# cmusphinx/pocketsphinx

Hardware: NVIDIA H100
Metric: frames/sec senone-eval+Viterbi (higher is better)
Workload: dtype f32->i16/i32

## Files before the change

### pocketsphinx_b200/csrc/psb_ptm_tc.cu

```cuda
#include "psb_gau.cuh"
#include "psb_internal.cuh"

#include <algorithm>
#include <cmath>
#include <cstring>

namespace {

constexpr int TC_ROWS = 128;
constexpr int TC_K = 32;
constexpr int TC_CAP = 18;
constexpr float TC_ERR = 1.0f / 262144.f;

enum {
    ST_ROWS, ST_FILTER_ALONE, ST_EXACT_DIST, ST_TIE_FLAGS,
    ST_OVER_CAP,
    ST_LANE_OVER,
    ST_FALLBACK_LISTED, ST_FALLBACK_ALL,
    ST_SPLIT,
    ST_FAIL_GAP, ST_FAIL_STRADDLE, ST_FAIL_SIGN, ST_FAIL_SAT,
    ST_N
};
constexpr size_t TC_CHECK_BYTES = 16 + 8 * ST_N;

__device__ __forceinline__ float to_tf32(float x)
{
    unsigned r;
    asm("cvt.rna.tf32.f32 %0, %1;" : "=r"(r) : "f"(x));
    return __uint_as_float(r);
}

struct Top5 {
    int s[5];
    unsigned c;
    int c4;
    int n;
};

__device__ __forceinline__ void top5_insert(Top5 &t, int s, int c)
{
    int p = 0;
#pragma unroll
    for (int j = 0; j < 5; ++j) p += (j < t.n && t.s[j] >= s) ? 1 : 0;
    if (p >= 5) return;
#pragma unroll
    for (int j = 4; j >= 1; --j)
        if (j > p) t.s[j] = t.s[j - 1];
#pragma unroll
    for (int j = 0; j < 5; ++j)
        if (j == p) t.s[j] = s;
    if (p < 4) {
        const unsigned lowmask = p == 0 ? 0u : (0xffffffffu >> (32 - 8 * p));
        t.c4 = (int)(t.c >> 24);
        t.c = (t.c & lowmask) | ((unsigned)c << (8 * p)) | ((t.c << 8) & ~(lowmask | (0xffu << (8 * p))));
    }
    else
        t.c4 = c;
    if (t.n < 5) ++t.n;
}

constexpr int WG_ROWS = 64;
constexpr int WG_SLOTS = (TC_CAP + 1) * WG_ROWS * 4;
constexpr int WG_EXTRA = WG_SLOTS * 8 + WG_ROWS * 4 * 4 + WG_ROWS * 4 + 2 * WG_ROWS * 4 + WG_ROWS * 20;

__device__ __forceinline__ uint64_t wgmma_desc(const void *p, unsigned lbo_bytes, unsigned sbo_bytes)
{
    const uint64_t a = (uint64_t)(((unsigned)__cvta_generic_to_shared(p) >> 4) & 0x3fffu);
    return a | ((uint64_t)((lbo_bytes >> 4) & 0x3fffu) << 16) | ((uint64_t)((sbo_bytes >> 4) & 0x3fffu) << 32);
}

template <int R>
__device__ __forceinline__ void wgmma_fence_regs(float (&d)[R])
{
#pragma unroll
    for (int i = 0; i < R; ++i) asm volatile("" : "+f"(d[i])::"memory");
}

__device__ __forceinline__ void warpgroup_bar(int id) { asm volatile("bar.sync %0, 128;" ::"r"(id) : "memory"); }

template <int N>
struct Wgmma;
#define PSB_ACC8(i) "+f"(d[i]), "+f"(d[i + 1]), "+f"(d[i + 2]), "+f"(d[i + 3]), "+f"(d[i + 4]), "+f"(d[i + 5]), "+f"(d[i + 6]), "+f"(d[i + 7])
template <> struct Wgmma<64> {
    static __device__ __forceinline__ void mma(float (&d)[32], uint64_t a, uint64_t b, int accumulate)
    {
        asm volatile("{\n.reg .pred p;\nsetp.ne.b32 p, %34, 0;\nwgmma.mma_async.sync.aligned.m64n64k8.f32.tf32.tf32 {"
        "%0,%1,%2,%3,%4,%5,%6,%7,%8,%9,%10,%11,%12,%13,%14,%15,%16,%17,%18,%19,%20,%21,%22,%23,%24,%25,%26,%27,%28,%29,"
        "%30,%31"
        "}, %32, %33, p, 1, 1;\n}\n"
        : PSB_ACC8(0), PSB_ACC8(8), PSB_ACC8(16), PSB_ACC8(24)
        : "l"(a), "l"(b), "r"(accumulate));
    }
};
template <> struct Wgmma<128> {
    static __device__ __forceinline__ void mma(float (&d)[64], uint64_t a, uint64_t b, int accumulate)
    {
        asm volatile("{\n.reg .pred p;\nsetp.ne.b32 p, %66, 0;\nwgmma.mma_async.sync.aligned.m64n128k8.f32.tf32.tf32 {"
        "%0,%1,%2,%3,%4,%5,%6,%7,%8,%9,%10,%11,%12,%13,%14,%15,%16,%17,%18,%19,%20,%21,%22,%23,%24,%25,%26,%27,%28,%29,"
        "%30,%31,%32,%33,%34,%35,%36,%37,%38,%39,%40,%41,%42,%43,%44,%45,%46,%47,%48,%49,%50,%51,%52,%53,%54,%55,%56,"
        "%57,%58,%59,%60,%61,%62,%63"
        "}, %64, %65, p, 1, 1;\n}\n"
        : PSB_ACC8(0), PSB_ACC8(8), PSB_ACC8(16), PSB_ACC8(24), PSB_ACC8(32), PSB_ACC8(40), PSB_ACC8(48), PSB_ACC8(56)
        : "l"(a), "l"(b), "r"(accumulate));
    }
};
template <> struct Wgmma<256> {
    static __device__ __forceinline__ void mma(float (&d)[128], uint64_t a, uint64_t b, int accumulate)
    {
        asm volatile("{\n.reg .pred p;\nsetp.ne.b32 p, %130, 0;\nwgmma.mma_async.sync.aligned.m64n256k8.f32.tf32.tf32 {"
        "%0,%1,%2,%3,%4,%5,%6,%7,%8,%9,%10,%11,%12,%13,%14,%15,%16,%17,%18,%19,%20,%21,%22,%23,%24,%25,%26,%27,%28,%29,"
        "%30,%31,%32,%33,%34,%35,%36,%37,%38,%39,%40,%41,%42,%43,%44,%45,%46,%47,%48,%49,%50,%51,%52,%53,%54,%55,%56,"
        "%57,%58,%59,%60,%61,%62,%63,%64,%65,%66,%67,%68,%69,%70,%71,%72,%73,%74,%75,%76,%77,%78,%79,%80,%81,%82,%83,"
        "%84,%85,%86,%87,%88,%89,%90,%91,%92,%93,%94,%95,%96,%97,%98,%99,%100,%101,%102,%103,%104,%105,%106,%107,%108,"
        "%109,%110,%111,%112,%113,%114,%115,%116,%117,%118,%119,%120,%121,%122,%123,%124,%125,%126,%127"
        "}, %128, %129, p, 1, 1;\n}\n"
        : PSB_ACC8(0), PSB_ACC8(8), PSB_ACC8(16), PSB_ACC8(24), PSB_ACC8(32), PSB_ACC8(40), PSB_ACC8(48), PSB_ACC8(56),
          PSB_ACC8(64), PSB_ACC8(72), PSB_ACC8(80), PSB_ACC8(88), PSB_ACC8(96), PSB_ACC8(104), PSB_ACC8(112),
          PSB_ACC8(120)
        : "l"(a), "l"(b), "r"(accumulate));
    }
};
#undef PSB_ACC8

template <int FL, int ND, bool CHECK>
__global__ void __launch_bounds__(2 * 128, 1)
ptm_wgmma_kernel(const float *__restrict__ feats, long long total, int D, const int32_t *__restrict__ featoff,
                 const int32_t *__restrict__ klist, const float *__restrict__ wumma, const float *__restrict__ cen,
                 const float *__restrict__ bnd, const float *__restrict__ rec, const size_t *__restrict__ rec_off,
                 int4 *__restrict__ out, unsigned *__restrict__ flags, long long flag_words, int K, int n_feat,
                 int tiles_per_cta, uint4 *__restrict__ items, unsigned *__restrict__ n_items, unsigned item_cap,
                 float *__restrict__ check, unsigned long long *__restrict__ stats)
{
    constexpr int RF = (1 + 2 * FL + 3) / 4 * 4;
    constexpr int NTL = ND / 8;
    constexpr int NPG = NTL / 8;
    constexpr unsigned FULL = 0xffffffffu;
    static_assert(2 * FL + 1 <= TC_K && (ND == 64 || ND == 128 || ND == 256), "shape");
    extern __shared__ __align__(128) unsigned char wg_smem[];
    const int tid = threadIdx.x, wg = tid >> 7, t = tid & 127, warp = t >> 5, lane = tid & 31;
    float *sW = reinterpret_cast<float *>(wg_smem);
    float *sX = sW + 2 * 8 * ND * 4 + wg * (2 * 8 * WG_ROWS * 4);
    unsigned char *ex = wg_smem + (size_t)2 * 8 * ND * 16 + 2 * (2 * 8 * WG_ROWS * 16) + (size_t)wg * WG_EXTRA;
    float2 *Pv = reinterpret_cast<float2 *>(ex);
    unsigned *Pm = reinterpret_cast<unsigned *>(Pv + WG_SLOTS);
    float *thrs = reinterpret_cast<float *>(Pm + WG_ROWS * 4);
    float *epsr = thrs + WG_ROWS;
    unsigned *Lc = reinterpret_cast<unsigned *>(epsr + 2 * WG_ROWS);

    const int k = klist[blockIdx.x];
    const int f = k % n_feat;
    {
        const float4 *src = reinterpret_cast<const float4 *>(wumma + (size_t)k * 2 * 8 * ND * 4);
        float4 *dst = reinterpret_cast<float4 *>(sW);
        for (int i = tid; i < 2 * 8 * ND; i += 2 * 128) dst[i] = src[i];
    }
    __syncthreads();
    const float *m = cen + (size_t)k * 16, *bb = bnd + (size_t)k * 32;
    const float *rc = rec + rec_off[k];
    const int r = t & (WG_ROWS - 1), half = t >> 6;
    const int g = lane >> 2, q4 = lane & 3;
    const int ra = warp * 16 + g, rb = ra + 8;

    float xn[FL];
    auto fetch = [&](long long row) {
        const float *p = feats + (row < total ? row : 0) * D + featoff[f];
#pragma unroll
        for (int j = 0; j < FL; ++j) xn[j] = row < total ? p[j] : 0.f;
    };
    auto prepare = [&](float *eps) {
        float v[TC_K];
        float S = bb[2 * FL];
#pragma unroll
        for (int j = 0; j < FL; ++j) {
            const float y = __fsub_rn(xn[j], m[j]);
            const float y2 = __fmul_rn(y, y);
            v[j] = y2;
            v[FL + j] = y;
            if (half == 0) {
                S = __fadd_ru(S, __fmul_ru(bb[j], y2));
                S = __fadd_ru(S, __fmul_ru(bb[FL + j], fabsf(y)));
            }
        }
        v[2 * FL] = 1.0f;
#pragma unroll
        for (int j = 2 * FL + 1; j < TC_K; ++j) v[j] = 0.f;
#pragma unroll
        for (int kc = 0; kc < 8; ++kc) {
            if ((kc & 1) != half) continue;
            float4 h, l;
            h.x = to_tf32(v[4 * kc]); h.y = to_tf32(v[4 * kc + 1]); h.z = to_tf32(v[4 * kc + 2]); h.w = to_tf32(v[4 * kc + 3]);
            l.x = to_tf32(__fsub_rn(v[4 * kc], h.x)); l.y = to_tf32(__fsub_rn(v[4 * kc + 1], h.y));
            l.z = to_tf32(__fsub_rn(v[4 * kc + 2], h.z)); l.w = to_tf32(__fsub_rn(v[4 * kc + 3], h.w));
            reinterpret_cast<float4 *>(sX)[kc * WG_ROWS + r] = h;
            reinterpret_cast<float4 *>(sX)[(8 + kc) * WG_ROWS + r] = l;
        }
        if (half == 0) eps[r] = __fadd_ru(__fmul_ru(S, TC_ERR), 2.0f);
        asm volatile("fence.proxy.async.shared::cta;" ::: "memory");
        warpgroup_bar(1 + wg);
    };
    float acc[ND / 2];
    auto gemm = [&]() {
#pragma unroll
        for (int i = 0; i < ND / 2; ++i) acc[i] = 0.f;
        wgmma_fence_regs(acc);
        asm volatile("wgmma.fence.sync.aligned;" ::: "memory");
#pragma unroll
        for (int pass = 0; pass < 3; ++pass) {
            const int ha = pass == 0 ? 1 : 0, hb = pass == 1 ? 1 : 0;
#pragma unroll
            for (int ks = 0; ks < 4; ++ks) {
                const uint64_t ad = wgmma_desc(sX + (size_t)(ha * 8 + 2 * ks) * WG_ROWS * 4, WG_ROWS * 16, 128);
                const uint64_t bd = wgmma_desc(sW + (size_t)(hb * 8 + 2 * ks) * ND * 4, ND * 16, 128);
                Wgmma<ND>::mma(acc, ad, bd, (pass | ks) ? 1 : 0);
            }
        }
        asm volatile("wgmma.commit_group.sync.aligned;" ::: "memory");
    };

    auto resolve = [&](const long long row0, const float *eps) {
        const int rr = t >> 1, h = t & 1;
        const long long row = row0 + rr;
        const bool valid = row < total;
        unsigned char *lb = reinterpret_cast<unsigned char *>(Lc + rr * 5);
        float a[5] = {-INFINITY, -INFINITY, -INFINITY, -INFINITY, -INFINITY};
        int c[5] = {0, 0, 0, 0, 0};
        int nl = 0;
        bool over = false;
        {
            const float thr = thrs[rr];
            auto cand = [&](float v, int col) {
                const bool p = v >= thr;
                if (p && nl < TC_CAP) lb[h ? TC_CAP - 1 - nl : nl] = (unsigned char)col;
                nl += p ? 1 : 0;
                v = p ? v : -INFINITY;
#pragma unroll
                for (int j = 0; j < 5; ++j) {
                    const bool s = v > a[j];
                    const float tv = a[j];
                    const int tc = c[j];
                    a[j] = s ? v : tv; c[j] = s ? col : tc;
                    v = s ? tv : v; col = s ? tc : col;
                }
            };
            unsigned m0 = Pm[rr * 4 + 2 * h], m1 = Pm[rr * 4 + 2 * h + 1];
            over = __popc(m0) > TC_CAP || __popc(m1) > TC_CAP;
            int j0 = 0, j1 = 0;
            while ((m0 | m1) != 0u) {
                const bool first = m0 != 0u;
                const unsigned msk = first ? m0 : m1;
                const int i = __ffs(msk) - 1, q = 2 * h + (first ? 0 : 1), j = first ? j0 : j1;
                const float2 v = Pv[j * WG_ROWS * 4 + rr * 4 + q];
                cand(v.x, 8 * i + 2 * q);
                cand(v.y, 8 * i + 2 * q + 1);
                if (first) { m0 = ++j0 < TC_CAP ? m0 & (m0 - 1u) : 0u; }
                else { m1 = ++j1 < TC_CAP ? m1 & (m1 - 1u) : 0u; }
            }
        }
        const int n1 = __shfl_xor_sync(FULL, nl, 1), n = nl + n1;
        over = __shfl_xor_sync(FULL, (int)over, 1) != 0 || over;
        {
            float b[5];
            int bc[5];
#pragma unroll
            for (int j = 0; j < 5; ++j) { b[j] = __shfl_xor_sync(FULL, a[j], 1); bc[j] = __shfl_xor_sync(FULL, c[j], 1); }
#pragma unroll
            for (int j = 0; j < 5; ++j)
                if (b[4 - j] > a[j]) { a[j] = b[4 - j]; c[j] = bc[4 - j]; }
            auto cmpx = [&](int i, int j) {
                if (a[j] > a[i]) { const float tv = a[i]; const int tc = c[i]; a[i] = a[j]; c[i] = c[j]; a[j] = tv; c[j] = tc; }
            };
            cmpx(0, 1); cmpx(3, 4); cmpx(2, 4); cmpx(2, 3); cmpx(1, 4); cmpx(0, 3); cmpx(0, 2); cmpx(1, 3); cmpx(1, 2);
        }
        const bool listed = n >= 5 && n <= TC_CAP && !over;
        const float ee = eps[rr];

        bool certain = listed;
        {
            const float gap = __fadd_ru(__fadd_ru(ee, ee), 1.0f);
            int qv[4];
            bool gap_ok = true, straddle_ok = true;
#pragma unroll
            for (int j = 0; j < 4; ++j) {
                gap_ok &= __fsub_rd(a[j], a[j + 1]) > gap;
                const int lo = __float2int_ru(__fsub_rd(a[j], ee)), hi = __float2int_ru(__fadd_ru(a[j], ee));
                straddle_ok &= (lo >> PSB_SENSCR_SHIFT) == (hi >> PSB_SENSCR_SHIFT);
                qv[j] = lo >> PSB_SENSCR_SHIFT;
            }
            const bool sign_ok = __fadd_ru(a[0], ee) < -2.0f, sat_ok = a[4] > -2.0e9f;
            certain &= gap_ok && straddle_ok && sign_ok && sat_ok;
            if (valid && h == 0) {
                if (CHECK) {
                    atomicMax(reinterpret_cast<int *>(check) + 1, n);
                    if (n > TC_CAP) atomicAdd(stats + ST_OVER_CAP, 1ull);
                    if (over) atomicAdd(stats + ST_LANE_OVER, 1ull);
                    if (listed) {
                        if (!gap_ok) atomicAdd(stats + ST_FAIL_GAP, 1ull);
                        if (!straddle_ok) atomicAdd(stats + ST_FAIL_STRADDLE, 1ull);
                        if (!sign_ok) atomicAdd(stats + ST_FAIL_SIGN, 1ull);
                        if (!sat_ok) atomicAdd(stats + ST_FAIL_SAT, 1ull);
                    }
                }
                if (certain) {
                    unsigned cb = 0, eb = 0;
#pragma unroll
                    for (int j = 0; j < 4; ++j) {
                        int ev = qv[0] - qv[j];
                        ev = ev > 255 ? 255 : ev;
                        cb |= (unsigned)c[j] << (8 * j);
                        eb |= (unsigned)ev << (8 * j);
                    }
                    out[row * K + k] = make_int4(qv[0], (int)cb, (int)eb, 0);
                    if (CHECK) { atomicAdd(stats, 1ull); atomicAdd(stats + 1, 1ull); }
                }
            }
        }
        __syncwarp();
        const bool doubt = valid && h == 0 && !certain;
        const int n0 = listed ? nl : 255, nb = listed ? n1 : 0;
        if (CHECK && doubt && listed && nl > 0 && n1 > 0) atomicAdd(stats + ST_SPLIT, 1ull);
        bool handled = false;
        if (items) {
            const unsigned need = __ballot_sync(FULL, doubt);
            if (need) {
                const int leader = __ffs(need) - 1;
                unsigned base = 0;
                if (lane == leader) base = atomicAdd(n_items, (unsigned)__popc(need));
                base = __shfl_sync(FULL, base, leader);
                const unsigned slot = base + (unsigned)__popc(need & ((1u << lane) - 1u));
                if (doubt && slot < item_cap) {
                    const unsigned *w = Lc + rr * 5;
                    items[2 * (size_t)slot] = make_uint4((unsigned)row, (unsigned)k | ((unsigned)n0 << 16) | ((unsigned)nb << 24), w[0], w[1]);
                    items[2 * (size_t)slot + 1] = make_uint4(w[2], w[3], w[4], (unsigned)(row >> 32));
                    handled = true;
                    if (CHECK) atomicAdd(stats, 1ull);
                }
            }
        }
        if (doubt && !handled) {
            float x[FL];
            const float *px = feats + row * D + featoff[f];
#pragma unroll
            for (int j = 0; j < FL; ++j) x[j] = px[j];
            Top5 top;
            top.n = 0; top.c = 0u; top.c4 = 0;
#pragma unroll
            for (int j = 0; j < 5; ++j) top.s[j] = INT_MIN;
            const int cnt_l = listed ? n : ND;
            if (CHECK) atomicAdd(stats + (listed ? ST_FALLBACK_LISTED : ST_FALLBACK_ALL), 1ull);
            for (int i = 0; i < cnt_l; ++i) {
                const int cw = listed ? (int)lb[i < n0 ? i : i - n0 + TC_CAP - nb] : i;
                const float d = gau_dist<FL>(reinterpret_cast<const float4 *>(rc + (size_t)cw * RF), x);
                top5_insert(top, f2i_clamped(d), cw);
            }
            const bool distinct = top.n >= 5 && top.s[0] > top.s[1] && top.s[1] > top.s[2] && top.s[2] > top.s[3] && top.s[3] > top.s[4];
            const int tp = top.s[0] >> PSB_SENSCR_SHIFT;
            unsigned eb = 0;
#pragma unroll
            for (int j = 0; j < 4; ++j) {
                int ev = tp - (top.s[j] >> PSB_SENSCR_SHIFT);
                ev = ev > 255 ? 255 : ev;
                eb |= (unsigned)ev << (8 * j);
            }
            out[row * K + k] = make_int4(tp, (int)top.c, (int)eb, 0);
            if (!distinct) atomicOr(&flags[(size_t)k * flag_words + (row >> 5)], 1u << (row & 31));
            if (CHECK) { atomicAdd(stats, 1ull); atomicAdd(stats + 2, (unsigned long long)cnt_l); if (!distinct) atomicAdd(stats + 3, 1ull); }
        }
    };

    long long row0 = (long long)blockIdx.y * tiles_per_cta * TC_ROWS + wg * WG_ROWS;
    if (row0 >= total) return;
    fetch(row0 + r);
    prepare(epsr);
    int buf = 0;
    for (int tile = 0;; ++tile, buf ^= 1, row0 += TC_ROWS) {
        gemm();
        const bool more = tile + 1 < tiles_per_cta && row0 + TC_ROWS < total;
        if (more) fetch(row0 + TC_ROWS + r);
        if (tile > 0) {
            resolve(row0 - TC_ROWS, epsr + (buf ^ 1) * WG_ROWS);
            warpgroup_bar(1 + wg);
        }
        const float *eps = epsr + buf * WG_ROWS;
        asm volatile("wgmma.wait_group.sync.aligned 0;" ::: "memory");
        wgmma_fence_regs(acc);

        float gma[8], gmb[8];
#pragma unroll
        for (int q = 0; q < 8; ++q) {
            float a = -INFINITY, b = -INFINITY;
#pragma unroll
            for (int i = q * NPG; i < (q + 1) * NPG; ++i) {
                a = fmaxf(fmaxf(a, acc[4 * i]), acc[4 * i + 1]);
                b = fmaxf(fmaxf(b, acc[4 * i + 2]), acc[4 * i + 3]);
            }
            a = fmaxf(a, __shfl_xor_sync(FULL, a, 1)); a = fmaxf(a, __shfl_xor_sync(FULL, a, 2));
            b = fmaxf(b, __shfl_xor_sync(FULL, b, 1)); b = fmaxf(b, __shfl_xor_sync(FULL, b, 2));
            gma[q] = a; gmb[q] = b;
        }
        auto fifth = [](float (&gm)[8]) {
            auto cmpx = [&](int i, int j) { const float hi = fmaxf(gm[i], gm[j]); gm[j] = fminf(gm[i], gm[j]); gm[i] = hi; };
#pragma unroll
            for (int o = 0; o < 8; o += 4) { cmpx(o, o + 1); cmpx(o + 2, o + 3); cmpx(o, o + 2); cmpx(o + 1, o + 3); cmpx(o + 1, o + 2); }
            return fmaxf(fmaxf(fminf(gm[0], gm[7]), fminf(gm[1], gm[6])), fmaxf(fminf(gm[2], gm[5]), fminf(gm[3], gm[4])));
        };
        const float e_a = eps[ra], e_b = eps[rb];
        const float thra = __fsub_rd(__fsub_rd(floorf(__fsub_rd(fifth(gma), e_a)), 1.0f), e_a);
        const float thrb = __fsub_rd(__fsub_rd(floorf(__fsub_rd(fifth(gmb), e_b)), 1.0f), e_b);
        {
            constexpr int SS = WG_ROWS * 4;
            int oa = ra * 4 + q4, ob = rb * 4 + q4;
            const int lim_a = oa + TC_CAP * SS, lim_b = ob + TC_CAP * SS;
            unsigned ma = 0u, mb = 0u;
#pragma unroll
            for (int i = 0; i < NTL; ++i) {
                const bool pa = fmaxf(acc[4 * i], acc[4 * i + 1]) >= thra;
                const bool pb = fmaxf(acc[4 * i + 2], acc[4 * i + 3]) >= thrb;
                if (pa) Pv[oa] = make_float2(acc[4 * i], acc[4 * i + 1]);
                if (pb) Pv[ob] = make_float2(acc[4 * i + 2], acc[4 * i + 3]);
                oa = pa ? min(oa + SS, lim_a) : oa;
                ob = pb ? min(ob + SS, lim_b) : ob;
                ma |= pa ? 1u << i : 0u;
                mb |= pb ? 1u << i : 0u;
            }
            Pm[ra * 4 + q4] = ma;
            Pm[rb * 4 + q4] = mb;
            if (q4 == 0) { thrs[ra] = thra; thrs[rb] = thrb; }
        }
        if (CHECK) {
            float worst = 0.f;
#pragma unroll
            for (int h = 0; h < 2; ++h) {
                const int rr = h ? rb : ra;
                if (row0 + rr >= total) continue;
                const float *px = feats + (row0 + rr) * D + featoff[f];
                const float er = eps[rr];
#pragma unroll
                for (int i = 0; i < NTL; ++i)
#pragma unroll
                    for (int e = 0; e < 2; ++e) {
                        const float *rp = rc + (size_t)(8 * i + 2 * q4 + e) * RF;
                        float d = rp[0];
                        for (int j = 0; j < FL; ++j) {
                            const float df = __fsub_rn(px[j], rp[1 + 2 * j]);
                            d = __fsub_rn(d, __fmul_rn(__fmul_rn(df, df), rp[2 + 2 * j]));
                        }
                        worst = fmaxf(worst, __fdividef(fabsf(acc[4 * i + 2 * h + e] - d), er));
                    }
            }
            atomicMax(reinterpret_cast<int *>(check), __float_as_int(worst));
        }
        warpgroup_bar(1 + wg);
        if (!more) break;
        prepare(epsr + (buf ^ 1) * WG_ROWS);
    }
    resolve(row0, epsr + buf * WG_ROWS);
}

template <int FL>
__global__ void __launch_bounds__(128)
ptm_tc_exact_kernel(const float *__restrict__ feats, int D, const int32_t *__restrict__ featoff, const uint4 *__restrict__ items,
                    const unsigned *__restrict__ n_items, unsigned item_cap, const float *__restrict__ rec,
                    const size_t *__restrict__ rec_off, int4 *__restrict__ out, unsigned *__restrict__ flags, long long flag_words,
                    int K, int n_feat, int nd, unsigned long long *__restrict__ stats)
{
    constexpr int RF = (1 + 2 * FL + 3) / 4 * 4;
    const unsigned count = min(*n_items, item_cap);
    for (unsigned i = blockIdx.x * blockDim.x + threadIdx.x; i < count; i += gridDim.x * blockDim.x) {
        const uint4 a = items[2 * (size_t)i], b = items[2 * (size_t)i + 1];
        const long long row = (long long)a.x | ((long long)b.w << 32);
        const int k = (int)(a.y & 0xffffu), n0 = (int)((a.y >> 16) & 0xffu), n1 = (int)(a.y >> 24);
        const unsigned wv[5] = {a.z, a.w, b.x, b.y, b.z};
        const float *px = feats + row * D + featoff[k % n_feat];
        const float *rc = rec + rec_off[k];
        float x[FL];
#pragma unroll
        for (int j = 0; j < FL; ++j) x[j] = px[j];
        Top5 top;
        top.n = 0; top.c = 0u; top.c4 = 0;
#pragma unroll
        for (int j = 0; j < 5; ++j) top.s[j] = INT_MIN;
        const int cnt = n0 == 255 ? nd : n0 + n1;
        for (int q = 0; q < cnt; ++q) {
            const int pos = q < n0 ? q : q - n0 + TC_CAP - n1;
            const int cw = n0 == 255 ? q : (int)((wv[pos >> 2] >> (8 * (pos & 3))) & 0xffu);
            const float d = gau_dist<FL>(reinterpret_cast<const float4 *>(rc + (size_t)cw * RF), x);
            top5_insert(top, f2i_clamped(d), cw);
        }
        const bool distinct = top.n >= 5 && top.s[0] > top.s[1] && top.s[1] > top.s[2] && top.s[2] > top.s[3] && top.s[3] > top.s[4];
        const int tp = top.s[0] >> PSB_SENSCR_SHIFT;
        unsigned eb = 0;
#pragma unroll
        for (int j = 0; j < 4; ++j) {
            int ev = tp - (top.s[j] >> PSB_SENSCR_SHIFT);
            ev = ev > 255 ? 255 : ev;
            eb |= (unsigned)ev << (8 * j);
        }
        out[row * K + k] = make_int4(tp, (int)top.c, (int)eb, 0);
        if (!distinct) atomicOr(&flags[(size_t)k * flag_words + (row >> 5)], 1u << (row & 31));
        if (stats) { atomicAdd(stats + 2, (unsigned long long)cnt); if (!distinct) atomicAdd(stats + 3, 1ull); }
    }
}

template <int FL, int NDW>
__global__ void __launch_bounds__(128)
ptm_fixup_warp_kernel(const float *__restrict__ feats, int D, const int32_t *__restrict__ featoff, const int32_t *__restrict__ utt_off,
                      int n_utt, const float *__restrict__ rec, const size_t *__restrict__ rec_off, int4 *__restrict__ out,
                      const unsigned *__restrict__ flags, long long flag_words, int K, int n_feat)
{
    constexpr int RF = (1 + 2 * FL + 3) / 4 * 4;
    constexpr unsigned FULL = 0xffffffffu;
    const long long id = ((long long)blockIdx.x * blockDim.x + threadIdx.x) >> 5;
    const int lane = threadIdx.x & 31;
    if (id >= (long long)n_utt * K) return;
    const int u = (int)(id / K), k = (int)(id % K);
    const int f = k % n_feat;
    const long long f0 = utt_off[u], f1 = utt_off[u + 1];
    if (f1 <= f0) return;
    const unsigned *fl = flags + (size_t)k * flag_words;
    const float *rc = rec + rec_off[k];
    for (long long w0 = f0 >> 5; w0 <= (f1 - 1) >> 5; w0 += 32) {
        const long long wd_l = w0 + lane;
        unsigned mine = wd_l <= ((f1 - 1) >> 5) ? fl[wd_l] : 0u;
        unsigned any = __ballot_sync(FULL, mine != 0u);
        while (any) {
            const int wl = __ffs(any) - 1;
            any &= any - 1;
            unsigned bits = __shfl_sync(FULL, mine, wl);
            while (bits) {
                const int b = __ffs(bits) - 1;
                bits &= bits - 1;
                const long long row = (w0 + wl) * 32 + b;
                if (row < f0 || row >= f1) continue;
                const float *px = feats + row * D + featoff[f];
                float x[FL];
#pragma unroll
                for (int j = 0; j < FL; ++j) x[j] = px[j];
                float d[NDW];
#pragma unroll
                for (int q = 0; q < NDW; ++q) d[q] = gau_dist<FL>(reinterpret_cast<const float4 *>(rc + (size_t)(lane + 32 * q) * RF), x);
                auto dist_of = [&](int c) {
                    float v = d[0];
#pragma unroll
                    for (int q = 1; q < NDW; ++q) v = (c >> 5) == q ? d[q] : v;
                    return __shfl_sync(FULL, v, c & 31);
                };
                const unsigned seeds = row == f0 ? 0x03020100u : (unsigned)out[(row - 1) * K + k].y;
                int cw[4], sc[4];
#pragma unroll
                for (int i = 0; i < 4; ++i) {
                    const int c = (seeds >> (8 * i)) & 0xff;
                    const int s = f2i_clamped(dist_of(c));
                    int p = 0;
#pragma unroll
                    for (int j = 0; j < i; ++j) p += (s > sc[j]) ? 0 : 1;
#pragma unroll
                    for (int j = 2; j >= 0; --j)
                        if (j < i && j >= p) { sc[j + 1] = sc[j]; cw[j + 1] = cw[j]; }
#pragma unroll
                    for (int j = 0; j < 4; ++j)
                        if (j == p) { sc[j] = s; cw[j] = c; }
                }
                const float th0 = (float)sc[3];
#pragma unroll
                for (int q = 0; q < NDW; ++q) {
                    unsigned cand = __ballot_sync(FULL, d[q] >= th0);
                    while (cand) {
                        const int l = __ffs(cand) - 1;
                        cand &= cand - 1;
                        const int c = l + 32 * q;
                        const float dv = __shfl_sync(FULL, d[q], l);
                        if (!(dv >= (float)sc[3])) continue;
                        if (cw[0] == c || cw[1] == c || cw[2] == c || cw[3] == c) continue;
                        const int s = f2i_clamped(dv);
                        int p = 0;
#pragma unroll
                        for (int j = 0; j < 3; ++j) p += (s >= sc[j]) ? 0 : 1;
#pragma unroll
                        for (int j = 2; j >= 0; --j)
                            if (j >= p) { sc[j + 1] = sc[j]; cw[j + 1] = cw[j]; }
#pragma unroll
                        for (int j = 0; j < 4; ++j)
                            if (j == p) { sc[j] = s; cw[j] = c; }
                    }
                }
                if (lane == 0) {
                    const int tp = sc[0] >> PSB_SENSCR_SHIFT;
                    unsigned cb = 0, eb = 0;
#pragma unroll
                    for (int j = 0; j < 4; ++j) {
                        int ev = tp - (sc[j] >> PSB_SENSCR_SHIFT);
                        ev = ev > 255 ? 255 : ev;
                        cb |= (unsigned)cw[j] << (8 * j);
                        eb |= (unsigned)ev << (8 * j);
                    }
                    out[row * K + k] = make_int4(tp, (int)cb, (int)eb, 0);
                }
                __syncwarp();
            }
        }
    }
}

float round_tf32_host(float x)
{
    uint32_t u;
    memcpy(&u, &x, 4);
    if ((u & 0x7f800000u) == 0x7f800000u) return x;
    u = (u + 0x1000u) & ~0x1fffu;
    float r;
    memcpy(&r, &u, 4);
    return r;
}

template <int FL, int ND>
int launch_wgmma(psb_batch_t *b, const float *d_feats, long long total, const int32_t *d_klist, int n_k, const int32_t *d_featoff,
               bool check)
{
    psb_model_t *m = b->m;
    const size_t smem = (size_t)2 * 8 * ND * 16 + 2 * ((size_t)2 * 8 * WG_ROWS * 16 + WG_EXTRA);
    const long long tiles = (total + TC_ROWS - 1) / TC_ROWS;
    const int n_sm = psb_sm_count(m->device);
    int per_sm = 1;
    PSB_CUDA(cudaFuncSetAttribute(ptm_wgmma_kernel<FL, ND, false>, cudaFuncAttributeMaxDynamicSharedMemorySize, (int)smem));
    PSB_CUDA(cudaOccupancyMaxActiveBlocksPerMultiprocessor(&per_sm, ptm_wgmma_kernel<FL, ND, false>, TC_ROWS * 2, smem));
    int tpc = 1;
    while (tpc < 32 && (tiles / (tpc * 2)) * n_k >= (long long)n_sm * std::max(per_sm, 1) * 4) tpc *= 2;
    PSB_REQUIRE((tiles + tpc - 1) / tpc <= 65535, "too many frames for one launch of the tensor-core filter");
    const dim3 grid((unsigned)n_k, (unsigned)((tiles + tpc - 1) / tpc));
    b->tc_last_tpc = tpc;
    b->tc_last_ctas = grid.y;
    float *chk = b->d_tc_check;
    unsigned long long *stats = reinterpret_cast<unsigned long long *>(b->d_tc_check + 4);
    if (check) {
        auto kern = ptm_wgmma_kernel<FL, ND, true>;
        PSB_CUDA(cudaFuncSetAttribute(kern, cudaFuncAttributeMaxDynamicSharedMemorySize, (int)smem));
        kern<<<grid, TC_ROWS * 2, smem, b->stream>>>(d_feats, total, m->sumlen, d_featoff, d_klist, m->d_tc_wumma, m->d_tc_cen, m->d_tc_bnd,
                                                m->d_rec, m->d_rec_off, b->d_topn, b->d_tc_flags, (long long)b->tc_flag_words, m->K,
                                                m->n_feat, tpc, b->d_tc_items, b->d_tc_nitems, b->tc_item_cap, chk, stats);
    }
    else {
        auto kern = ptm_wgmma_kernel<FL, ND, false>;
        PSB_CUDA(cudaFuncSetAttribute(kern, cudaFuncAttributeMaxDynamicSharedMemorySize, (int)smem));
        kern<<<grid, TC_ROWS * 2, smem, b->stream>>>(d_feats, total, m->sumlen, d_featoff, d_klist, m->d_tc_wumma, m->d_tc_cen, m->d_tc_bnd,
                                                m->d_rec, m->d_rec_off, b->d_topn, b->d_tc_flags, (long long)b->tc_flag_words, m->K,
                                                m->n_feat, tpc, b->d_tc_items, b->d_tc_nitems, b->tc_item_cap, nullptr, nullptr);
    }
    PSB_LAUNCH_CHECK();
    if (b->d_tc_items) {
        const unsigned blocks = (unsigned)std::min<size_t>(((size_t)b->tc_item_cap + 127) / 128, (size_t)n_sm * 64);
        ptm_tc_exact_kernel<FL><<<blocks, 128, 0, b->stream>>>(d_feats, m->sumlen, d_featoff, b->d_tc_items, b->d_tc_nitems, b->tc_item_cap,
                                                              m->d_rec, m->d_rec_off, b->d_topn, b->d_tc_flags, (long long)b->tc_flag_words,
                                                              m->K, m->n_feat, ND, check ? stats : nullptr);
        PSB_LAUNCH_CHECK();
    }
    return PSB_OK;
}

}

int psb_tc_prepare(psb_model_t *m, const float *hm, const float *hv, const float *hd)
{
    m->tc_ok = false;
    if (m->kind != PSB_KIND_PTM || m->fixed_point || m->topn != 4) return PSB_OK;
    if (m->n_density != 64 && m->n_density != 128 && m->n_density != 256) return PSB_OK;
    for (int f = 0; f < m->n_feat; ++f)
        if (m->featlen[f] != 13) return PSB_OK;
    const int nd = m->n_density, FL = 13, K = m->K;
    std::vector<float> cen((size_t)K * 16, 0.f), bnd((size_t)K * 32, 0.f);
    std::vector<float> wu((size_t)K * 2 * 8 * nd * 4, 0.f);
    std::vector<double> W((size_t)TC_K * nd);
    for (int cb = 0; cb < m->n_mgau; ++cb)
        for (int f = 0; f < m->n_feat; ++f) {
            const int k = cb * m->n_feat + f;
            const size_t src = ((size_t)cb * m->sumlen + m->featoff[f]) * nd;
            const float *mu = hm + src, *vv = hv + src, *dt = hd + (size_t)k * nd;
            float *c = cen.data() + (size_t)k * 16, *bb = bnd.data() + (size_t)k * 32;
            for (int j = 0; j < FL; ++j) {
                double s = 0;
                for (int q = 0; q < nd; ++q) s += mu[(size_t)q * FL + j];
                c[j] = (float)(s / nd);
            }
            std::fill(W.begin(), W.end(), 0.0);
            double cmax = 0;
            for (int q = 0; q < nd; ++q) {
                double c0 = dt[q], quad = 0;
                for (int j = 0; j < FL; ++j) {
                    const double v = vv[(size_t)q * FL + j], mp = (double)mu[(size_t)q * FL + j] - (double)c[j];
                    W[(size_t)j * nd + q] = -v;
                    W[(size_t)(FL + j) * nd + q] = 2.0 * v * mp;
                    quad += std::fabs(v) * mp * mp;
                    c0 -= v * mp * mp;
                    bb[j] = std::max(bb[j], (float)std::fabs(v));
                    bb[FL + j] = std::max(bb[FL + j], (float)std::fabs(2.0 * v * mp));
                }
                W[(size_t)(2 * FL) * nd + q] = c0;
                cmax = std::max(cmax, std::fabs((double)dt[q]) + quad);
            }
            bb[2 * FL] = (float)(cmax * 1.0001);
            for (int j = 0; j < 2 * FL; ++j) bb[j] = std::nextafter(bb[j] * 1.0001f, INFINITY);
            float *u = wu.data() + (size_t)k * 2 * 8 * nd * 4;
            for (int kk = 0; kk < TC_K; ++kk)
                for (int q = 0; q < nd; ++q) {
                    const float v = (float)W[(size_t)kk * nd + q], h = round_tf32_host(v);
                    u[((size_t)(kk >> 2) * nd + q) * 4 + (kk & 3)] = h;
                    u[((size_t)(8 + (kk >> 2)) * nd + q) * 4 + (kk & 3)] = round_tf32_host(v - h);
                }
            for (int i = 0; i < 32; ++i)
                if (!std::isfinite(bb[i])) return PSB_OK;
        }
    if (!m->d_tc_wumma) {
        PSB_CUDA(cudaMalloc(&m->d_tc_wumma, wu.size() * sizeof(float)));
        PSB_CUDA(cudaMalloc(&m->d_tc_cen, cen.size() * sizeof(float)));
        PSB_CUDA(cudaMalloc(&m->d_tc_bnd, bnd.size() * sizeof(float)));
    }
    PSB_CUDA(cudaMemcpy(m->d_tc_wumma, wu.data(), wu.size() * sizeof(float), cudaMemcpyHostToDevice));
    PSB_CUDA(cudaMemcpy(m->d_tc_cen, cen.data(), cen.size() * sizeof(float), cudaMemcpyHostToDevice));
    PSB_CUDA(cudaMemcpy(m->d_tc_bnd, bnd.data(), bnd.size() * sizeof(float), cudaMemcpyHostToDevice));
    m->tc_ok = true;
    return PSB_OK;
}

bool psb_tc_usable(const psb_batch_t *b)
{
    const psb_model_t *m = b->m;
    return m->tc_ok && m->ds_ratio == 1 && b->topn_variant >= 6;
}

int psb_launch_ptm_tc(psb_batch_t *b, const float *d_feats, const int32_t *utt_off, int32_t n_utt, const int32_t *d_klist,
                      const int32_t *d_featoff)
{
    psb_model_t *m = b->m;
    const long long total = utt_off[n_utt];
    const size_t fw = (size_t)((total + 31) / 32) + 1;
    if (fw * m->K > b->tc_flag_cap) {
        cudaFree(b->d_tc_flags);
        b->d_tc_flags = nullptr;
        b->tc_flag_cap = fw * m->K + fw * m->K / 8;
        PSB_CUDA(cudaMalloc(&b->d_tc_flags, b->tc_flag_cap * 4));
    }
    if ((size_t)n_utt + 1 > b->uttoff_cap) {
        if (b->d_uttoff) cudaFree(b->d_uttoff);
        b->d_uttoff = nullptr;
        b->uttoff_cap = (size_t)n_utt + 1 + 64;
        PSB_CUDA(cudaMalloc(&b->d_uttoff, b->uttoff_cap * sizeof(int32_t)));
    }
    if (!b->d_tc_check) {
        PSB_CUDA(cudaMalloc(&b->d_tc_check, TC_CHECK_BYTES));
        PSB_CUDA(cudaMemsetAsync(b->d_tc_check, 0, TC_CHECK_BYTES, b->stream));
    }
    {
        const size_t want = std::max<size_t>(4096, (size_t)total * m->K / 4);
        if (want > b->tc_item_cap || !b->d_tc_items) {
            cudaFree(b->d_tc_items);
            b->d_tc_items = nullptr;
            if (!b->d_tc_nitems) PSB_CUDA(cudaMalloc(&b->d_tc_nitems, 4));
            b->tc_item_cap = (unsigned)std::min<size_t>(want + want / 8, 0x7fffffffu);
            PSB_CUDA(cudaMalloc(&b->d_tc_items, (size_t)b->tc_item_cap * 32));
        }
        PSB_CUDA(cudaMemsetAsync(b->d_tc_nitems, 0, 4, b->stream));
    }
    b->tc_flag_words = fw;
    PSB_CUDA(cudaMemsetAsync(b->d_tc_flags, 0, fw * m->K * 4, b->stream));
    PSB_CUDA(cudaMemcpyAsync(b->d_uttoff, utt_off, ((size_t)n_utt + 1) * sizeof(int32_t), cudaMemcpyHostToDevice, b->stream));
    static const bool check = [] { const char *v = getenv("PSB_TC_CHECK"); return v && atoi(v) != 0; }();
    int rc;
    switch (m->n_density) {
    case 256: rc = launch_wgmma<13, 256>(b, d_feats, total, d_klist, m->K, d_featoff, check); break;
    case 128: rc = launch_wgmma<13, 128>(b, d_feats, total, d_klist, m->K, d_featoff, check); break;
    default: rc = launch_wgmma<13, 64>(b, d_feats, total, d_klist, m->K, d_featoff, check); break;
    }
    if (rc) return rc;
    const long long chains = (long long)n_utt * m->K;
    const unsigned blocks = (unsigned)((chains * 32 + 127) / 128);
#define PSB_FIXW(NDW) ptm_fixup_warp_kernel<13, NDW><<<blocks, 128, 0, b->stream>>>(d_feats, m->sumlen, d_featoff, b->d_uttoff, n_utt, \
        m->d_rec, m->d_rec_off, b->d_topn, b->d_tc_flags, (long long)fw, m->K, m->n_feat)
    if (m->n_density == 256) PSB_FIXW(8);
    else if (m->n_density == 128) PSB_FIXW(4);
    else PSB_FIXW(2);
#undef PSB_FIXW
    PSB_LAUNCH_CHECK();
    return PSB_OK;
}

extern "C" int psb_batch_tc_check(psb_batch_t *b, float *ratio, int32_t *max_candidates, int64_t *stats4)
{
    PSB_REQUIRE(b && ratio && max_candidates, "psb_batch_tc_check: null argument");
    *ratio = 0.f; *max_candidates = 0;
    if (stats4) stats4[0] = stats4[1] = stats4[2] = stats4[3] = 0;
    if (!b->d_tc_check) return PSB_OK;
    PSB_CUDA(cudaSetDevice(b->m->device));
    PSB_CUDA(cudaStreamSynchronize(b->stream));
    unsigned char h[64];
    PSB_CUDA(cudaMemcpy(h, b->d_tc_check, sizeof(h), cudaMemcpyDeviceToHost));
    memcpy(ratio, h, 4);
    memcpy(max_candidates, h + 4, 4);
    if (stats4) memcpy(stats4, h + 16, 32);
    return PSB_OK;
}

extern "C" int psb_batch_tc_counters(psb_batch_t *b, int64_t *out, int32_t n)
{
    PSB_REQUIRE(b && (out || n == 0) && n >= 0, "psb_batch_tc_counters: bad argument");
    static_assert(ST_N + 2 == PSB_TC_N_COUNTERS, "psb200.h lists every counter");
    int64_t v[PSB_TC_N_COUNTERS] = {0};
    if (b->d_tc_check) {
        PSB_CUDA(cudaSetDevice(b->m->device));
        PSB_CUDA(cudaStreamSynchronize(b->stream));
        PSB_CUDA(cudaMemcpy(v, reinterpret_cast<unsigned char *>(b->d_tc_check) + 16, 8 * ST_N, cudaMemcpyDeviceToHost));
    }
    v[ST_N] = b->tc_last_tpc;
    v[ST_N + 1] = b->tc_last_ctas;
    memcpy(out, v, sizeof(int64_t) * (size_t)std::min<int32_t>(n, PSB_TC_N_COUNTERS));
    return PSB_OK;
}
```

Baseline: 9.948 million.

## Use three warpgroups per CTA for small-ND tensor-core filter kernel

The wgmma filter kernel now launches a variable number of warpgroups per CTA: three when ND ≤ 128, two otherwise. Each warpgroup strides over 64-row half-tiles by the warpgroup count instead of owning a fixed half of every 128-row tile. Shared memory, the weight copy loop and the launch config are sized to match. The aim is more concurrent MMA and resolve work per SM, since the per-CTA weight tile is shared, at the cost of more shared memory and registers per CTA and possibly uneven work across warpgroups.

```diff
diff --git a/pocketsphinx_b200/csrc/psb_ptm_tc.cu b/pocketsphinx_b200/csrc/psb_ptm_tc.cu
--- a/pocketsphinx_b200/csrc/psb_ptm_tc.cu
+++ b/pocketsphinx_b200/csrc/psb_ptm_tc.cu
@@ -59,6 +59,7 @@
     if (t.n < 5) ++t.n;
 }
 
+__host__ __device__ constexpr int tc_warpgroups(int nd) { return nd > 128 ? 2 : 3; }
 constexpr int WG_ROWS = 64;
 constexpr int WG_SLOTS = (TC_CAP + 1) * WG_ROWS * 4;
 constexpr int WG_EXTRA = WG_SLOTS * 8 + WG_ROWS * 4 * 4 + WG_ROWS * 4 + 2 * WG_ROWS * 4 + WG_ROWS * 20;
@@ -123,7 +124,7 @@
 #undef PSB_ACC8
 
 template <int FL, int ND, bool CHECK>
-__global__ void __launch_bounds__(2 * 128, 1)
+__global__ void __launch_bounds__(tc_warpgroups(ND) * 128, 1)
 ptm_wgmma_kernel(const float *__restrict__ feats, long long total, int D, const int32_t *__restrict__ featoff,
                  const int32_t *__restrict__ klist, const float *__restrict__ wumma, const float *__restrict__ cen,
                  const float *__restrict__ bnd, const float *__restrict__ rec, const size_t *__restrict__ rec_off,
@@ -134,13 +135,14 @@
     constexpr int RF = (1 + 2 * FL + 3) / 4 * 4;
     constexpr int NTL = ND / 8;
     constexpr int NPG = NTL / 8;
+    constexpr int WG_N = tc_warpgroups(ND);
     constexpr unsigned FULL = 0xffffffffu;
     static_assert(2 * FL + 1 <= TC_K && (ND == 64 || ND == 128 || ND == 256), "shape");
     extern __shared__ __align__(128) unsigned char wg_smem[];
     const int tid = threadIdx.x, wg = tid >> 7, t = tid & 127, warp = t >> 5, lane = tid & 31;
     float *sW = reinterpret_cast<float *>(wg_smem);
     float *sX = sW + 2 * 8 * ND * 4 + wg * (2 * 8 * WG_ROWS * 4);
-    unsigned char *ex = wg_smem + (size_t)2 * 8 * ND * 16 + 2 * (2 * 8 * WG_ROWS * 16) + (size_t)wg * WG_EXTRA;
+    unsigned char *ex = wg_smem + (size_t)2 * 8 * ND * 16 + WG_N * (2 * 8 * WG_ROWS * 16) + (size_t)wg * WG_EXTRA;
     float2 *Pv = reinterpret_cast<float2 *>(ex);
     unsigned *Pm = reinterpret_cast<unsigned *>(Pv + WG_SLOTS);
     float *thrs = reinterpret_cast<float *>(Pm + WG_ROWS * 4);
@@ -152,7 +154,7 @@
     {
         const float4 *src = reinterpret_cast<const float4 *>(wumma + (size_t)k * 2 * 8 * ND * 4);
         float4 *dst = reinterpret_cast<float4 *>(sW);
-        for (int i = tid; i < 2 * 8 * ND; i += 2 * 128) dst[i] = src[i];
+        for (int i = tid; i < 2 * 8 * ND; i += WG_N * 128) dst[i] = src[i];
     }
     __syncthreads();
     const float *m = cen + (size_t)k * 16, *bb = bnd + (size_t)k * 32;
@@ -367,17 +369,20 @@
         }
     };
 
-    long long row0 = (long long)blockIdx.y * tiles_per_cta * TC_ROWS + wg * WG_ROWS;
-    if (row0 >= total) return;
+    constexpr long long STEP = (long long)WG_N * WG_ROWS;
+    const int n_half = 2 * tiles_per_cta;
+    int hx = wg;
+    long long row0 = (long long)blockIdx.y * tiles_per_cta * TC_ROWS + (long long)hx * WG_ROWS;
+    if (hx >= n_half || row0 >= total) return;
     fetch(row0 + r);
     prepare(epsr);
     int buf = 0;
-    for (int tile = 0;; ++tile, buf ^= 1, row0 += TC_ROWS) {
+    for (bool first = true;; first = false, buf ^= 1, hx += WG_N, row0 += STEP) {
         gemm();
-        const bool more = tile + 1 < tiles_per_cta && row0 + TC_ROWS < total;
-        if (more) fetch(row0 + TC_ROWS + r);
-        if (tile > 0) {
-            resolve(row0 - TC_ROWS, epsr + (buf ^ 1) * WG_ROWS);
+        const bool more = hx + WG_N < n_half && row0 + STEP < total;
+        if (more) fetch(row0 + STEP + r);
+        if (!first) {
+            resolve(row0 - STEP, epsr + (buf ^ 1) * WG_ROWS);
             warpgroup_bar(1 + wg);
         }
         const float *eps = epsr + buf * WG_ROWS;
@@ -617,12 +622,13 @@
                bool check)
 {
     psb_model_t *m = b->m;
-    const size_t smem = (size_t)2 * 8 * ND * 16 + 2 * ((size_t)2 * 8 * WG_ROWS * 16 + WG_EXTRA);
+    constexpr int WG_N = tc_warpgroups(ND), threads = WG_N * 128;
+    const size_t smem = (size_t)2 * 8 * ND * 16 + WG_N * ((size_t)2 * 8 * WG_ROWS * 16 + WG_EXTRA);
     const long long tiles = (total + TC_ROWS - 1) / TC_ROWS;
     const int n_sm = psb_sm_count(m->device);
     int per_sm = 1;
     PSB_CUDA(cudaFuncSetAttribute(ptm_wgmma_kernel<FL, ND, false>, cudaFuncAttributeMaxDynamicSharedMemorySize, (int)smem));
-    PSB_CUDA(cudaOccupancyMaxActiveBlocksPerMultiprocessor(&per_sm, ptm_wgmma_kernel<FL, ND, false>, TC_ROWS * 2, smem));
+    PSB_CUDA(cudaOccupancyMaxActiveBlocksPerMultiprocessor(&per_sm, ptm_wgmma_kernel<FL, ND, false>, threads, smem));
     int tpc = 1;
     while (tpc < 32 && (tiles / (tpc * 2)) * n_k >= (long long)n_sm * std::max(per_sm, 1) * 4) tpc *= 2;
     PSB_REQUIRE((tiles + tpc - 1) / tpc <= 65535, "too many frames for one launch of the tensor-core filter");
@@ -634,14 +640,14 @@
     if (check) {
         auto kern = ptm_wgmma_kernel<FL, ND, true>;
         PSB_CUDA(cudaFuncSetAttribute(kern, cudaFuncAttributeMaxDynamicSharedMemorySize, (int)smem));
-        kern<<<grid, TC_ROWS * 2, smem, b->stream>>>(d_feats, total, m->sumlen, d_featoff, d_klist, m->d_tc_wumma, m->d_tc_cen, m->d_tc_bnd,
+        kern<<<grid, threads, smem, b->stream>>>(d_feats, total, m->sumlen, d_featoff, d_klist, m->d_tc_wumma, m->d_tc_cen, m->d_tc_bnd,
                                                 m->d_rec, m->d_rec_off, b->d_topn, b->d_tc_flags, (long long)b->tc_flag_words, m->K,
                                                 m->n_feat, tpc, b->d_tc_items, b->d_tc_nitems, b->tc_item_cap, chk, stats);
     }
     else {
         auto kern = ptm_wgmma_kernel<FL, ND, false>;
         PSB_CUDA(cudaFuncSetAttribute(kern, cudaFuncAttributeMaxDynamicSharedMemorySize, (int)smem));
-        kern<<<grid, TC_ROWS * 2, smem, b->stream>>>(d_feats, total, m->sumlen, d_featoff, d_klist, m->d_tc_wumma, m->d_tc_cen, m->d_tc_bnd,
+        kern<<<grid, threads, smem, b->stream>>>(d_feats, total, m->sumlen, d_featoff, d_klist, m->d_tc_wumma, m->d_tc_cen, m->d_tc_bnd,
                                                 m->d_rec, m->d_rec_off, b->d_topn, b->d_tc_flags, (long long)b->tc_flag_words, m->K,
                                                 m->n_feat, tpc, b->d_tc_items, b->d_tc_nitems, b->tc_item_cap, nullptr, nullptr);
     }
```

Measured after the change: 9.966 million (median of 6 runs). About the same (+0.2%).
